# nz0001na/MorphGANformer

Hardware: AMD Instinct MI355X
Metric: latent-projection iters/sec @1024^2, k=17 latents (higher is better)
Workload: dtype f32; 1 GPU; configs[1]: single 1024x1024 face per GPU, Wing+LPIPS(squeeze)+MSE literal-mode projection step, noise_mode=random, seeded synthetic weights/targets/landmarks; k=17, z_dim=32, targets_per_gpu=1, parallelism=pair-sharded x1, graph_replay=True, loss_generator_overlap=True, steps_per_forward=32

## Files before the change

include/mgf.h:

```cpp
#ifndef MGF_H_
#define MGF_H_

#include <stdint.h>

#ifdef __cplusplus
extern "C" {
#endif

typedef void* mgf_stream_t;

enum { MGF_OK = 0, MGF_EINVAL = -1, MGF_EUNSUPPORTED = -2, MGF_ELAUNCH = -3, MGF_ETOOBIG = -4 };
enum { MGF_F32 = 0, MGF_F64 = 1, MGF_F16 = 2 };
enum { MGF_FILTER_SEPARABLE = 2 };
enum { MGF_FILTER_LARGE = 4 };
enum { MGF_ACT_LINEAR = 1, MGF_ACT_RELU = 2, MGF_ACT_LRELU = 3, MGF_ACT_TANH = 4, MGF_ACT_SIGMOID = 5,
       MGF_ACT_ELU = 6, MGF_ACT_SELU = 7, MGF_ACT_SOFTPLUS = 8, MGF_ACT_SWISH = 9,
       MGF_ACT_RELU_POST = 10 };

const char* mgf_last_error(void);
int mgf_version(void);
int mgf_device_ok(void);

int mgf_bias_act(void* y, const void* x, const void* b, const void* xref, const void* yref, const void* dy,
                 int dtype, int64_t numel, int64_t step_b, int64_t size_b,
// ... 270 lines not shown
} mgf_attn_bwd_job;
int mgf_style_demod_bwd_multi(float* dwg, const mgf_style_bwd_job* jobs_dev, int32_t njobs, int32_t n, int32_t wdim, int32_t max_channels,
                              mgf_stream_t stream);
int mgf_attn_values_bwd_multi(float* dyc, const mgf_attn_bwd_job* jobs_dev, int32_t njobs, int32_t n, int32_t t, int32_t wdim,
                              mgf_stream_t stream);
int mgf_latent_bwd_multi(float* dwg, const mgf_style_bwd_job* style_jobs_dev, int32_t n_style_jobs, float* dyc,
                         const mgf_attn_bwd_job* attn_jobs_dev, int32_t n_attn_jobs, int32_t n, int32_t t, int32_t wdim, int32_t max_channels,
                         mgf_stream_t stream);
int32_t mgf_attn_values_grad_slices(int32_t n, int32_t c, int32_t f, int32_t t);
int64_t mgf_attn_grad_job_bytes(void);
int mgf_attn_grad_multi(const void* jobs_dev, int32_t njobs, int32_t n, int32_t grad_blocks, int32_t dot_blocks, int32_t reduce_blocks,
                        mgf_stream_t stream);
int mgf_latent_grad_gather(float* dw, const float* dwg, int32_t n_style_jobs, const float* dyc, int32_t n_attn_jobs, int32_t n, int32_t k,
                           int32_t wdim, float scale, mgf_stream_t stream);
int64_t mgf_mapping_bwd_scratch_floats(int32_t k, int32_t dim, int32_t n_res_layers);
int mgf_mapping_backward(float* dz, const float* dw, const float* z, const float* params, float* scratch, int32_t n, int32_t k,
                         int32_t dim, int32_t n_res_layers, int32_t normalize_global, mgf_stream_t stream);
int mgf_mapping_forward_save(float* w, const float* z, const float* params, float* scratch, int32_t n, int32_t k, int32_t dim,
                             int32_t n_res_layers, int32_t normalize_global, mgf_stream_t stream);
int mgf_mapping_backward_saved(float* dz, const float* dw, const float* z, const float* params, float* scratch, int32_t n, int32_t k,
                               int32_t dim, int32_t n_res_layers, int32_t normalize_global, mgf_stream_t stream);

int mgf_lpips_layer_bwd_f32(float* df0, const float* f0, const float* f1_unit, const float* lin, int32_t n, int32_t c, int64_t hw,
                            int64_t f1_batch_stride, float scale, int32_t accumulate, mgf_stream_t stream);
int mgf_lpips_layer_bwd_relu_f32(float* dz_a, float* dz_b, const float* dy, const float* f0, const float* f1_unit, const float* lin,
                                 int32_t n, int32_t c, int32_t c_split, int64_t hw, int64_t f1_batch_stride, float scale,
                                 mgf_stream_t stream);
int mgf_lpips_layer_stats_f32(float* out, float* stats, const float* f0, const float* f1_unit, const float* lin, int32_t n, int32_t c,
                              int64_t hw, int64_t f1_batch_stride, int32_t accumulate, float* scratch, mgf_stream_t stream);
int mgf_lpips_layer_defer_f32(float* scratch, float* stats, const float* f0, const float* f1_unit, const float* lin, int32_t n, int32_t c, int64_t hw,
                              int64_t f1_batch_stride, int32_t* nparts_out, mgf_stream_t stream);
int mgf_lpips_finish_taps_f32(float* out, const float* scratch, int64_t set_stride_floats, int32_t ntaps, const int32_t* nparts, const float* scales,
                              int32_t n, int32_t accumulate, mgf_stream_t stream);
int mgf_lpips_layer_bwd_relu_stats_f32(float* dz_a, float* dz_b, const float* dy, const float* f0, const float* f1_unit, const float* lin,
                                       const float* stats, int32_t n, int32_t c, int32_t c_split, int64_t hw, int64_t f1_batch_stride,
                                       float scale, mgf_stream_t stream);
int mgf_relu_bwd_split_f32(float* dz_a, float* dz_b, const float* dy, const float* y, int32_t n, int32_t c, int32_t c_split, int64_t hw,
                           mgf_stream_t stream);
int mgf_maxpool3x3s2_ceil_idx_f32(float* y, uint8_t* idx, const float* x, int32_t nc, int32_t in_h, int32_t in_w, int32_t out_h,
                                  int32_t out_w, mgf_stream_t stream);
int mgf_maxpool3x3s2_ceil_bwd_idx_f32(float* dx, const float* dy, const uint8_t* idx, int32_t nc, int32_t in_h, int32_t in_w, int32_t out_h,
                                      int32_t out_w, mgf_stream_t stream);
int mgf_maxpool3x3s2_ceil_bwd_f32(float* dx, const float* dy, const float* x, int32_t nc, int32_t in_h, int32_t in_w, int32_t out_h,
                                  int32_t out_w, mgf_stream_t stream);
int mgf_maxpool_s2_floor_bwd_f32(float* dx, const float* dy, const float* x, int32_t nc, int32_t in_h, int32_t in_w, int32_t ksize,
                                 mgf_stream_t stream);
int mgf_mse_grad_f32(float* d, const float* a, const float* b, int32_t n, int64_t numel, int64_t b_batch_stride, float scale,
                     int32_t accumulate, mgf_stream_t stream);

int mgf_lpips_layer_defer_weighted_f32(float* scratch, float* stats, const float* f0, const float* f1_unit, const float* lin, const float* wmap,
                                       int32_t n, int32_t c, int64_t hw, int64_t f1_batch_stride, int64_t w_batch_stride, int32_t* nparts_out,
                                       mgf_stream_t stream);
int mgf_lpips_layer_bwd_weighted_f32(float* df0, const float* f0, const float* f1_unit, const float* lin, const float* wmap, int32_t n, int32_t c,
                                     int64_t hw, int64_t f1_batch_stride, int64_t w_batch_stride, float scale, int32_t accumulate,
                                     mgf_stream_t stream);
int mgf_lpips_layer_bwd_relu_stats_weighted_f32(float* dz_a, float* dz_b, const float* dy, const float* f0, const float* f1_unit, const float* lin,
                                                const float* stats, const float* wmap, int32_t n, int32_t c, int32_t c_split, int64_t hw,
                                                int64_t f1_batch_stride, int64_t w_batch_stride, float scale, mgf_stream_t stream);
int mgf_mse_weighted_f32(float* out, const float* a, const float* b, const float* wmap, int32_t n, int32_t c, int64_t hw, int64_t b_batch_stride,
                         int64_t w_batch_stride, float scale, int32_t accumulate, float* scratch, mgf_stream_t stream);
int mgf_mse_weighted_grad_f32(float* d, const float* a, const float* b, const float* wmap, int32_t n, int32_t c, int64_t hw,
                              int64_t b_batch_stride, int64_t w_batch_stride, float scale, int32_t accumulate, mgf_stream_t stream);

int mgf_prelu_bwd_f32(float* dx, const float* dy, const float* y, const float* slope, int32_t n, int32_t c, int64_t hw, mgf_stream_t stream);
int mgf_linear_bwd_f32(float* dx, const float* dy, const float* w, int32_t n, int32_t in_features, int32_t out_features, mgf_stream_t stream);
int mgf_resize_bilinear_bwd_f32(float* dx, const float* dy, int32_t nc, int32_t in_h, int32_t in_w, int32_t out_h, int32_t out_w,
// ... 57 lines not shown
```

morphganformer_amd/_lib.py:

```python
from __future__ import annotations

import ctypes as C
import os

import torch

HERE = os.path.dirname(os.path.abspath(__file__))
LIB_PATH = os.environ.get("MGF_LIB_PATH") or os.path.join(HERE, "libmgf_hip.so")

MGF_F32, MGF_F64, MGF_F16 = 0, 1, 2
ACT_IDS = {"linear": 1, "relu": 2, "lrelu": 3, "tanh": 4, "sigmoid": 5, "elu": 6, "selu": 7, "softplus": 8, "swish": 9,
           "relu_post": 10}
MAX_TAPS = 9

i32, i64, f32, f64, vp = C.c_int32, C.c_int64, C.c_float, C.c_double, C.c_void_p


class Epilogue(C.Structure):
    _fields_ = [("bias", vp), ("noise", vp), ("noise_strength", vp), ("noise_n", i32), ("act", i32), ("alpha", f32),
                ("gain", f32), ("residual", vp)]


class ConvDesc(C.Structure):
    _fields_ = [("n", i32), ("cin", i32), ("in_h", i32), ("in_w", i32), ("cout", i32), ("cout_pad", i32),
# ... 108 lines not shown
    "mgf_maxpool_s2_floor_f32": (C.c_int, [vp, vp, i32, i32, i32, i32, vp]),
    "mgf_maxpool3x3s2_ceil_f32": (C.c_int, [vp, vp, i32, i32, i32, i32, i32, vp]),
    "mgf_latent_perturb": (C.c_int, [vp, vp, vp, vp, vp, i32, i32, i64, vp]),
    "mgf_latent_perturb_mean": (C.c_int, [vp, vp, vp, vp, vp, i32, i32, i64, i32, vp]),
    "mgf_select_best": (C.c_int, [vp, vp, vp, vp, vp, i64, vp, vp, vp, f64, f32, vp, vp, i32, i32, vp, vp, i32, vp, vp, vp]),
    "mgf_keep_improvements": (C.c_int, [vp, vp, i64, vp, i32, vp]),
    "mgf_to_uint8_hwc": (C.c_int, [vp, vp, i32, i32, i32, vp]),
    "mgf_reference_gray_scratch_floats": (i64, []),
    "mgf_reference_gray_u8": (C.c_int, [vp, vp, i32, i32, i32, vp, vp]),
    "mgf_bwd_chunks": (i32, [i64]),
    "mgf_layer_act_bwd_f32": (C.c_int, [vp, vp, vp, vp, vp, vp, vp, vp, i32, i32, i32, i64, f32, f32, vp]),
    "mgf_channel_dot_f32": (C.c_int, [vp, vp, vp, i32, i32, i64, vp]),
    "mgf_style_grad_f32": (C.c_int, [vp, vp, vp, vp, vp, i32, i32, i64, i32, vp]),
    "mgf_style_grad_act_bwd_f32": (C.c_int, [vp, vp, vp, vp, vp, vp, vp, vp, vp, i32, vp, vp, vp, i32, i32, i32, i64, f32, f32, vp]),
    "mgf_style_act_fir_tiles": (i32, [i32, i32]),
    "mgf_style_act_fir_bwd_f32": (C.c_int, [vp, vp, vp, vp, vp, vp, vp, vp, vp, i32, vp, i32, f32, i32, i32, i32, i32, f32, f32, vp]),
    "mgf_layer_act_bwd_low_f32": (C.c_int, [vp, vp, vp, vp, vp, vp, i32, vp, vp, vp, i32, i32, i32, i64, f32, f32, vp]),
    "mgf_duplex_attention_bwd": (C.c_int, [vp, vp, vp, vp, vp, vp, vp, vp, i32, i32, i32, i32, vp]),
    "mgf_attn_values_grad": (C.c_int, [vp, vp, vp, i32, i32, i32, i32, vp]),
    "mgf_attn_values_grad_workspace_floats": (C.c_int64, [i32, i32]),
    "mgf_attn_values_grad_ws": (C.c_int, [vp, vp, vp, i32, i32, i32, i32, vp, i64, vp]),
    "mgf_style_demod_bwd_multi": (C.c_int, [vp, vp, i32, i32, i32, i32, vp]),
    "mgf_attn_values_bwd_multi": (C.c_int, [vp, vp, i32, i32, i32, i32, vp]),
    "mgf_attn_values_grad_slices": (i32, [i32, i32, i32, i32]),
    "mgf_attn_grad_job_bytes": (i64, []),
    "mgf_attn_grad_multi": (C.c_int, [vp, i32, i32, i32, i32, i32, vp]),
    "mgf_latent_bwd_multi": (C.c_int, [vp, vp, i32, vp, vp, i32, i32, i32, i32, i32, vp]),
    "mgf_latent_grad_gather": (C.c_int, [vp, vp, i32, vp, i32, i32, i32, i32, f32, vp]),
    "mgf_lpips_layer_bwd_f32": (C.c_int, [vp, vp, vp, vp, i32, i32, i64, i64, f32, i32, vp]),
    "mgf_lpips_layer_bwd_relu_f32": (C.c_int, [vp, vp, vp, vp, vp, vp, i32, i32, i32, i64, i64, f32, vp]),
    "mgf_lpips_layer_stats_f32": (C.c_int, [vp, vp, vp, vp, vp, i32, i32, i64, i64, i32, vp, vp]),
    "mgf_lpips_layer_defer_f32": (C.c_int, [vp, vp, vp, vp, vp, i32, i32, i64, i64, C.POINTER(i32), vp]),
    "mgf_lpips_finish_taps_f32": (C.c_int, [vp, vp, i64, i32, C.POINTER(i32), C.POINTER(f32), i32, i32, vp]),
    "mgf_lpips_layer_bwd_relu_stats_f32": (C.c_int, [vp, vp, vp, vp, vp, vp, vp, i32, i32, i32, i64, i64, f32, vp]),
    "mgf_relu_bwd_split_f32": (C.c_int, [vp, vp, vp, vp, i32, i32, i32, i64, vp]),
    "mgf_maxpool3x3s2_ceil_idx_f32": (C.c_int, [vp, vp, vp, i32, i32, i32, i32, i32, vp]),
    "mgf_maxpool3x3s2_ceil_bwd_idx_f32": (C.c_int, [vp, vp, vp, i32, i32, i32, i32, i32, vp]),
    "mgf_maxpool3x3s2_ceil_bwd_f32": (C.c_int, [vp, vp, vp, i32, i32, i32, i32, i32, vp]),
    "mgf_maxpool_s2_floor_bwd_f32": (C.c_int, [vp, vp, vp, i32, i32, i32, i32, vp]),
    "mgf_mse_grad_f32": (C.c_int, [vp, vp, vp, i32, i64, i64, f32, i32, vp]),
    "mgf_lpips_layer_defer_weighted_f32": (C.c_int, [vp, vp, vp, vp, vp, vp, i32, i32, i64, i64, i64, C.POINTER(i32), vp]),
    "mgf_lpips_layer_bwd_weighted_f32": (C.c_int, [vp, vp, vp, vp, vp, i32, i32, i64, i64, i64, f32, i32, vp]),
    "mgf_lpips_layer_bwd_relu_stats_weighted_f32": (C.c_int, [vp, vp, vp, vp, vp, vp, vp, vp, i32, i32, i32, i64, i64, i64, f32, vp]),
    "mgf_mse_weighted_f32": (C.c_int, [vp, vp, vp, vp, i32, i32, i64, i64, i64, f32, i32, vp, vp]),
    "mgf_mse_weighted_grad_f32": (C.c_int, [vp, vp, vp, vp, i32, i32, i64, i64, i64, f32, i32, vp]),
    "mgf_prelu_bwd_f32": (C.c_int, [vp, vp, vp, vp, i32, i32, i64, vp]),
    "mgf_linear_bwd_f32": (C.c_int, [vp, vp, vp, i32, i32, i32, vp]),
    "mgf_resize_bilinear_bwd_f32": (C.c_int, [vp, vp, i32, i32, i32, i32, i32, vp]),
    "mgf_face_crop_check": (C.c_int, [vp, i32, i32]),
    "mgf_face_crop_f32": (C.c_int, [vp, vp, vp, i32, i32, i32, i32, i32, i32, vp]),
    "mgf_face_crop_bwd_f32": (C.c_int, [vp, vp, vp, i32, i32, i32, i32, i32, i32, i32, vp]),
    "mgf_dwconv_f32": (C.c_int, [vp, vp, vp, vp, vp, vp, i32, i32, i32, i32, i32, i32, i32, i32, vp]),
    "mgf_dwconv_bwd_data_f32": (C.c_int, [vp, vp, vp, vp, vp, vp, vp, vp, i32, i32, i32, i32, i32, i32, i32, i32, vp]),
    "mgf_cv_warp_triangle_bytes": (i64, []),
    "mgf_cv_warp_triangles_f32": (C.c_int, [vp, vp, vp, vp, i32, i32, i32, i32, f32, vp]),
    "mgf_adam_step_f32": (C.c_int, [vp, vp, vp, vp, vp, vp, vp, vp, i64, i32, f32, f32, f32, f32, vp]),
    "mgf_adam_elementwise_f32": (C.c_int, [vp, vp, vp, vp, vp, vp, vp, vp, i64, i32, f32, f32, f32, f32, vp]),
    "mgf_noise_grad_f32": (C.c_int, [vp, vp, vp, i32, i64, i32, vp]),
    "mgf_noise_regularize_scratch_bytes": (i64, [i32]),
    "mgf_noise_regularize_f32": (C.c_int, [vp, vp, i32, f32, i32, vp, vp]),
    "mgf_noise_regularize_grad_f32": (C.c_int, [vp, vp, vp, i32, f32, i32, i32, vp, vp]),
    "mgf_noise_normalize_scratch_bytes": (i64, []),
    "mgf_noise_normalize_f32": (C.c_int, [vp, i64, vp, vp, i32, vp, vp]),
    "mgf_mapping_bwd_scratch_floats": (i64, [i32, i32, i32]),
    "mgf_mapping_backward": (C.c_int, [vp, vp, vp, vp, vp, i32, i32, i32, i32, i32, vp]),
    "mgf_mapping_forward_save": (C.c_int, [vp, vp, vp, vp, i32, i32, i32, i32, i32, vp]),
# ... 68 lines not shown
```

morphganformer_amd/csrc/losses.hip:

```cpp
#include "mgf_common.h"

namespace {

constexpr int RED_BLOCKS = 16384;

__device__ __forceinline__ float block_sum_256(float v, float* sm) {
    v = wave_sum(v);
    if ((threadIdx.x & 63) == 0) sm[threadIdx.x >> 6] = v;
    __syncthreads();
    float r = sm[0] + sm[1] + sm[2] + sm[3];
    __syncthreads();
    return r;
}

__global__ __launch_bounds__(256) void finish_kernel(float* out, const float* scratch, int nparts, float scale, int accumulate) {
    __shared__ float sm[4];
    const float* sc = scratch + (int64_t)blockIdx.x * RED_BLOCKS;
    float v = 0.f;
    for (int i = threadIdx.x; i < nparts; i += 256) v += sc[i];
    v = block_sum_256(v, sm);
    if (threadIdx.x == 0) out[blockIdx.x] = (accumulate ? out[blockIdx.x] : 0.f) + v * scale;
}

struct FinishSets { int nparts[8]; float scale[8]; };
__global__ __launch_bounds__(256) void finish_multi_kernel(float* out, const float* scratch, int64_t set_stride, int nsets, FinishSets fs, int accumulate) {
    __shared__ float sm[4];
    float acc = accumulate ? out[blockIdx.x] : 0.f;
    for (int t = 0; t < nsets; ++t) {
        const float* sc = scratch + (int64_t)t * set_stride + (int64_t)blockIdx.x * RED_BLOCKS;
        float v = 0.f;
        for (int i = threadIdx.x; i < fs.nparts[t]; i += 256) v += sc[i];
        v = block_sum_256(v, sm);
        acc = acc + v * fs.scale[t];
// ... 150 lines not shown
        redb[grp][px] = nb;
        redc[grp][px] = nc;
        __syncthreads();
        if (grp == 0 && valid) {
            float sb = 0.f, sc = 0.f;
#pragma unroll
            for (int g = 0; g < G; ++g) { sb += redb[g][px]; sc += redc[g][px]; }
            float* so = stats + (int64_t)nn * 3 * hw + i;
            so[0] = na; so[hw] = sb; so[2 * hw] = sc;
        }
    }
    if (MAP) {
        redb[grp][px] = d;
        __syncthreads();
        if (grp == 0 && valid) {
            float sd = 0.f;
#pragma unroll
            for (int g = 0; g < G; ++g) sd += redb[g][px];
            stats[(int64_t)nn * hw + i] = sd;
        }
        return;
    }
    if (WEIGHTED) {
        unsigned t = threadIdx.x;
        asm volatile("" : "+v"(t));
        const int64_t iw = (int64_t)blk * PXB + (int)(t % PXB);
        const __amdgpu_buffer_rsrc_t rw = __builtin_amdgcn_make_buffer_rsrc((void*)(wmap + (int64_t)nn * w_stride), 0, (int)plane_bytes, 0x00020000);
        d *= __builtin_bit_cast(float, __builtin_amdgcn_raw_buffer_load_b32(rw, 4u * (unsigned)(iw < hw ? iw : hw - 1), 0, 0));
    }
    const float acc = block_sum_256(valid ? d : 0.f, sm);
    if (threadIdx.x == 0) scratch[(int64_t)nn * RED_BLOCKS + blk] = acc;
}

template <bool UNIT_OUT>
int launch_lpips_layer(float* scratch, float* unit_out, const float* f0, const float* f1u, const float* lin, int n, int c, int64_t hw,
                       int64_t f1_stride, hipStream_t st, int* grid_out, float* stats = nullptr, float* map = nullptr,
                       const float* wmap = nullptr, int64_t w_stride = 0) {
    static const int pxb_env = [] { const char* e = mgf_knob("MGF_LPIPS_PXB"); return e ? atoi(e) : 0; }();
    const int pxb = pxb_env ? pxb_env
                  : (c <= 256 && (hw >= 65536 || (int64_t)n * mgf_cdiv(hw, 64) >= 1024)) ? 64
                  : (c > 384 && (int64_t)n * mgf_cdiv(hw, 32) >= 1024) ? 32 : 16;
    const int64_t grid64 = mgf_cdiv(hw, pxb);
    MGF_REQUIRE(grid64 <= RED_BLOCKS, MGF_ETOOBIG, "lpips_layer: %lld pixels per sample need %lld scratch floats (have %d per sample)",
                (long long)hw, (long long)grid64, RED_BLOCKS);
    MGF_REQUIRE(c <= 512, MGF_EUNSUPPORTED, "lpips_layer: at most 512 channels per tap (got %d)", c);
    MGF_REQUIRE((int64_t)c * hw < (1LL << 30), MGF_ETOOBIG, "lpips_layer: one sample's tap must stay below 4 GiB");
    MGF_REQUIRE(grid64 * n <= INT32_MAX - 8, MGF_ETOOBIG, "lpips_layer: too many workgroups");
    const int xcd_per = (int)mgf_cdiv(grid64 * n, 8);
    const dim3 grid((unsigned)(xcd_per * 8));
    *grid_out = (int)grid64;
#define MGF_LPIPS_LAUNCH(PXB, CPT)                                                                                                            \
    do {                                                                                                                                      \
        if (!UNIT_OUT && wmap && stats)                                                                                                       \
            hipLaunchKernelGGL((lpips_layer_kernel<PXB, CPT, false, true, false, true>), grid, dim3(256), 0, st, scratch, unit_out, f0, f1u,  \
                               lin, c, hw, f1_stride, n, (int)grid64, xcd_per, stats, wmap, w_stride);                                        \
        else if (!UNIT_OUT && wmap)                                                                                                           \
            hipLaunchKernelGGL((lpips_layer_kernel<PXB, CPT, false, false, false, true>), grid, dim3(256), 0, st, scratch, unit_out, f0, f1u, \
                               lin, c, hw, f1_stride, n, (int)grid64, xcd_per, nullptr, wmap, w_stride);                                      \
        else if (!UNIT_OUT && map)                                                                                                            \
            hipLaunchKernelGGL((lpips_layer_kernel<PXB, CPT, false, false, true>), grid, dim3(256), 0, st, scratch, unit_out, f0, f1u, lin, c,\
                               hw, f1_stride, n, (int)grid64, xcd_per, map, nullptr, 0);                                                      \
        else if (!UNIT_OUT && stats)                                                                                                          \
            hipLaunchKernelGGL((lpips_layer_kernel<PXB, CPT, false, true>), grid, dim3(256), 0, st, scratch, unit_out, f0, f1u, lin, c, hw,   \
                               f1_stride, n, (int)grid64, xcd_per, stats, nullptr, 0);                                                        \
        else                                                                                                                                  \
            hipLaunchKernelGGL((lpips_layer_kernel<PXB, CPT, UNIT_OUT>), grid, dim3(256), 0, st, scratch, unit_out, f0, f1u, lin, c, hw,      \
                               f1_stride, n, (int)grid64, xcd_per, nullptr, nullptr, 0);                                                      \
    } while (0)
    if (pxb == 64) {
        if (c <= 128) MGF_LPIPS_LAUNCH(64, 32); else if (c <= 256) MGF_LPIPS_LAUNCH(64, 64); else MGF_LPIPS_LAUNCH(64, 128);
    } else if (pxb == 32) {
        if (c <= 128) MGF_LPIPS_LAUNCH(32, 16); else if (c <= 256) MGF_LPIPS_LAUNCH(32, 32); else MGF_LPIPS_LAUNCH(32, 64);
    } else {
        if (c <= 128) MGF_LPIPS_LAUNCH(16, 8); else if (c <= 256) MGF_LPIPS_LAUNCH(16, 16); else MGF_LPIPS_LAUNCH(16, 32);
    }
#undef MGF_LPIPS_LAUNCH
    return MGF_OK;
}

__global__ __launch_bounds__(256) void wing_kernel(double* out, const double* pred, const double* target, int64_t numel, double omega,
                                                   double epsilon, const int32_t* pred_step, int max_row) {
    __shared__ double sm[4];
    int row = (pred_step ? *pred_step : 0) + (int)blockIdx.x;
    if (max_row >= 0 && row > max_row) row = max_row;
    pred += (int64_t)row * numel;
    const double cc = omega - omega * log(1.0 + omega / epsilon);
    double acc = 0.0;
    for (int64_t i = threadIdx.x; i < numel; i += 256) {
        double dlt = fabs(target[i] - pred[i]);
        acc += dlt < omega ? omega * log(1.0 + dlt / epsilon) : dlt - cc;
    }
    acc = wave_sum(acc);
    if ((threadIdx.x & 63) == 0) sm[threadIdx.x >> 6] = acc;
    __syncthreads();
    if (threadIdx.x == 0) out[blockIdx.x] = (sm[0] + sm[1] + sm[2] + sm[3]) / (double)numel;
}

__global__ __launch_bounds__(256) void awing_kernel(double* out, const double* pred, const double* target, int64_t numel, double omega,
                                                    double theta, double epsilon, double alpha, const int32_t* pred_step, int max_row) {
    __shared__ double sm[4];
    int row = (pred_step ? *pred_step : 0) + (int)blockIdx.x;
    if (max_row >= 0 && row > max_row) row = max_row;
    pred += (int64_t)row * numel;
    double acc = 0.0;
    for (int64_t i = threadIdx.x; i < numel; i += 256) {
        const double y = target[i];
        const double dlt = fabs(y - pred[i]);
        const double pw = alpha - y;
        if (dlt < theta) {
            acc += omega * log(1.0 + pow(dlt / omega, pw));
        } else {
            const double tp = pow(theta / epsilon, pw);
// ... 300 lines not shown
    if (rc != MGF_OK) return rc;
    MGF_CHECK_LAUNCH("lpips_unit");
    return MGF_OK;
}

extern "C" int mgf_lpips_layer_f32(float* out, const float* f0, const float* f1_unit, const float* lin, int32_t n, int32_t c, int64_t hw,
                                   int64_t f1_batch_stride, int32_t accumulate, float* scratch, mgf_stream_t stream) {
    return mgf_lpips_layer_stats_f32(out, nullptr, f0, f1_unit, lin, n, c, hw, f1_batch_stride, accumulate, scratch, stream);
}

extern "C" int mgf_lpips_layer_stats_f32(float* out, float* stats, const float* f0, const float* f1_unit, const float* lin, int32_t n, int32_t c,
                                         int64_t hw, int64_t f1_batch_stride, int32_t accumulate, float* scratch, mgf_stream_t stream) {
    MGF_REQUIRE(out && f0 && f1_unit && lin && scratch && n >= 1 && n <= 65535 && c >= 1 && hw >= 1, MGF_EINVAL, "lpips_layer: bad arguments");
    hipStream_t st = (hipStream_t)stream;
    int grid = 0;
    const int rc = launch_lpips_layer<false>(scratch, nullptr, f0, f1_unit, lin, n, c, hw, f1_batch_stride, st, &grid, stats);
    if (rc != MGF_OK) return rc;
    hipLaunchKernelGGL(finish_kernel, dim3(n), dim3(256), 0, st, out, scratch, grid, 1.0f / (float)hw, accumulate);
    MGF_CHECK_LAUNCH("lpips_layer");
    return MGF_OK;
}

extern "C" int mgf_lpips_layer_defer_f32(float* scratch, float* stats, const float* f0, const float* f1_unit, const float* lin, int32_t n, int32_t c,
                                         int64_t hw, int64_t f1_batch_stride, int32_t* nparts_out, mgf_stream_t stream) {
    MGF_REQUIRE(scratch && f0 && f1_unit && lin && nparts_out && n >= 1 && n <= 65535 && c >= 1 && hw >= 1, MGF_EINVAL, "lpips_layer_defer: bad arguments");
    int grid = 0;
    const int rc = launch_lpips_layer<false>(scratch, nullptr, f0, f1_unit, lin, n, c, hw, f1_batch_stride, (hipStream_t)stream, &grid, stats);
    if (rc != MGF_OK) return rc;
    *nparts_out = grid;
    MGF_CHECK_LAUNCH("lpips_layer_defer");
    return MGF_OK;
}

extern "C" int mgf_lpips_layer_defer_weighted_f32(float* scratch, float* stats, const float* f0, const float* f1_unit, const float* lin,
                                                  const float* wmap, int32_t n, int32_t c, int64_t hw, int64_t f1_batch_stride,
                                                  int64_t w_batch_stride, int32_t* nparts_out, mgf_stream_t stream) {
    MGF_REQUIRE(scratch && f0 && f1_unit && lin && wmap && nparts_out && n >= 1 && n <= 65535 && c >= 1 && hw >= 1 && w_batch_stride >= 0, MGF_EINVAL,
                "lpips_layer_defer_weighted: bad arguments");
    int grid = 0;
    const int rc = launch_lpips_layer<false>(scratch, nullptr, f0, f1_unit, lin, n, c, hw, f1_batch_stride, (hipStream_t)stream, &grid, stats, nullptr,
                                             wmap, w_batch_stride);
    if (rc != MGF_OK) return rc;
    *nparts_out = grid;
    MGF_CHECK_LAUNCH("lpips_layer_defer_weighted");
    return MGF_OK;
}

extern "C" int mgf_lpips_finish_taps_f32(float* out, const float* scratch, int64_t set_stride_floats, int32_t ntaps, const int32_t* nparts,
                                         const float* scales, int32_t n, int32_t accumulate, mgf_stream_t stream) {
    MGF_REQUIRE(out && scratch && nparts && scales && ntaps >= 1 && ntaps <= 8 && n >= 1 && n <= 65535, MGF_EINVAL, "lpips_finish_taps: bad arguments (1..8 taps)");
    FinishSets fs;
    for (int t = 0; t < 8; ++t) { fs.nparts[t] = t < ntaps ? nparts[t] : 0; fs.scale[t] = t < ntaps ? scales[t] : 0.f; }
    for (int t = 0; t < ntaps; ++t) MGF_REQUIRE(nparts[t] >= 1 && nparts[t] <= RED_BLOCKS, MGF_EINVAL, "lpips_finish_taps: bad partial count");
    hipLaunchKernelGGL(finish_multi_kernel, dim3(n), dim3(256), 0, (hipStream_t)stream, out, scratch, set_stride_floats, ntaps, fs, accumulate);
    MGF_CHECK_LAUNCH("lpips_finish_taps");
    return MGF_OK;
}

extern "C" int mgf_lpips_layer_map_f32(float* map, const float* f0, const float* f1_unit, const float* lin, int32_t n, int32_t c, int64_t hw,
                                       int64_t f1_batch_stride, mgf_stream_t stream) {
    MGF_REQUIRE(map && f0 && f1_unit && lin && n >= 1 && n <= 65535 && c >= 1 && hw >= 1, MGF_EINVAL, "lpips_layer_map: bad arguments");
    int grid = 0;
    const int rc = launch_lpips_layer<false>(nullptr, nullptr, f0, f1_unit, lin, n, c, hw, f1_batch_stride, (hipStream_t)stream, &grid, nullptr, map);
    if (rc != MGF_OK) return rc;
    MGF_CHECK_LAUNCH("lpips_layer_map");
    return MGF_OK;
// ... 581 lines not shown
```

morphganformer_amd/lpips.py:

```python
from __future__ import annotations

import ctypes as C
import math
import os

import numpy as np
import torch

from . import _lib
from . import lpips_backbones as backbones
from .lpips_backbones import (ALEX_SPEC, CHNS, FIRES, NET_CHNS, POOLS, SCALE, SHIFT, SPECS, TAPS_AFTER, VGG_SPEC,
                              SequentialFeatures, SqueezeFeatures, _pool_out, load_backbone_state, random_backbone, random_squeeze_backbone)

WEIGHTS_DIR = os.path.join(os.path.dirname(os.path.abspath(__file__)), "weights")


def region_tap_weights(weight, sides):
    w = torch.as_tensor(weight).to(torch.float64)
    lead = w.shape[:-2]
    w4 = w.reshape(-1, 1, *w.shape[-2:])
    out = []
    for hh, ww in sides:
        wl = torch.nn.functional.adaptive_avg_pool2d(w4, (int(hh), int(ww)))
        wl = wl / wl.sum(dim=(2, 3), keepdim=True)
# ... 139 lines not shown
        if tuple(target_a.shape) != tuple(target_b.shape):
            raise ValueError(f"set_target_pair: the two targets differ in shape: {tuple(target_a.shape)} vs {tuple(target_b.shape)}")
        n = int(target_a.shape[0])
        al = np.asarray(alpha.detach().cpu() if isinstance(alpha, torch.Tensor) else alpha, dtype=np.float64).reshape(-1)
        if al.size not in (1, n) or not np.all((al >= 0.0) & (al <= 1.0)):
            raise ValueError(f"set_target_pair: alpha must be one value or {n} values in [0, 1] (got {alpha!r})")
        al = np.array(np.broadcast_to(al, (n,)))
        buf = self._pair_offset_buf
        if buf is None or buf.numel() != n:
            buf = self._pair_offset_buf = torch.zeros(n, dtype=torch.float32, device=self.device_)
        self.set_target(target_b)
        ub = [t.clone() for t in self._target_taps]
        self.distance_into(buf, target_a.float().contiguous())
        buf.mul_(torch.as_tensor(al * (1.0 - al), dtype=torch.float32, device=self.device_))
        self.set_target(target_a)
        for t, b in zip(self._target_taps, ub):
            for i in range(n):
                a = float(al[i])
                if a == 1.0:
                    t[i].copy_(b[i])
                elif a != 0.0:
                    t[i].mul_(1.0 - a).add_(b[i], alpha=a)
        self.pair_offset = buf

    def grad_into(self, dimg, scale=1.0, accumulate=False):
        f = self._last
        assert f is not None and tuple(dimg.shape) == (f.n, 3, *self._last_hw), "call distance_into(..., keep_taps=True) first"
        g = f.backward(self._target_taps, self.lins, scale, per_sample=self._target_n > 1, region=self._region_for(f.n, *self._last_hw))
        if not accumulate:
            dimg.zero_()
        dimg[:, :, :g.shape[2], :g.shape[3]].add_(g)
        return dimg

    def _forward_taps(self, pred, keep_taps=False, out=None, scalar=True):
        n, _, h, w = pred.shape
        f = self._features(n, h, w)
        assert self._target_taps is not None, "call set_target first"
        per_sample = self._target_n > 1
        assert not per_sample or self._target_n == n, f"{self._target_n} targets cannot pair with {n} candidates"
        if scalar:
            need = n * int(_lib.lib().mgf_reduce_scratch_floats())
            if self._scratch.numel() < need:
                self._scratch = torch.empty(need, dtype=torch.float32, device=self.device_)
            if out is None:
                out = torch.zeros(len(self.chns), n, dtype=torch.float32, device=self.device_)
        if keep_taps is not None:
            self._last, self._last_hw = (f, (h, w)) if keep_taps else (None, None)
        f.tap_stats = {}
        region = self._region_for(n, h, w) if scalar else None
        if scalar and self.fused_stem and not keep_taps and not per_sample and region is None:
            f.stem(pred.contiguous(), feat_ref=self._target_taps[0], lin=self.lins[0], dist_out=out if out.dim() == 1 else out[0],
                   scratch=self._scratch)
            taps = f(pred, from_pooled=True)
        else:
            taps = f(pred, argmax=True) if (keep_taps and self.net == "squeeze") else f(pred)
        return f, taps, per_sample, region, out

    def _defer_tap(self, i, a, scratch, stats, per_sample, region):
        n, c, hh, ww = a.shape
        L, st, hw, got = _lib.lib(), _lib.stream_ptr(), hh * ww, C.c_int32(0)
        maps = (a.data_ptr(), self._target_taps[i].data_ptr(), self.lins[i].data_ptr())
        if region is not None:
            _lib.check(L.mgf_lpips_layer_defer_weighted_f32(scratch.data_ptr(), _lib.ptr(stats), *maps, region[0][i].data_ptr(), n, c, hw,
                                                            c * hw if per_sample else 0, hw if region[1] > 1 else 0, C.byref(got), st),
                       "lpips_layer_weighted")
            return got.value, 1.0
        _lib.check(L.mgf_lpips_layer_defer_f32(scratch.data_ptr(), _lib.ptr(stats), *maps, n, c, hw, c * hw if per_sample else 0, C.byref(got), st),
                   "lpips_layer")
        return got.value, 1.0 / float(hw)

    def distance_into(self, out, pred, keep_taps=False):
        f, taps, per_sample, region, _ = self._forward_taps(pred, bool(keep_taps), out)
        n = pred.shape[0]
        L, st = _lib.lib(), _lib.stream_ptr()
        red = int(L.mgf_reduce_scratch_floats())
        ntaps = len(self.lins)
        if self._scratch.numel() < ntaps * n * red:
            self._scratch = torch.empty(ntaps * n * red, dtype=torch.float32, device=self.device_)
        nparts, scales, k, first_done = (C.c_int32 * 8)(), (C.c_float * 8)(), 0, False
        for i, a in enumerate(taps):
            if a is None:
                first_done = True
                continue
            hw = a.shape[2] * a.shape[3]
            stats = None
            if keep_taps and backbones.TAP_STATS:
                key = (i, n, hw)
                stats = self._stats.get(key)
                if stats is None:
                    stats = self._stats[key] = torch.empty(n, 3, hw, dtype=torch.float32, device=self.device_)
                f.tap_stats[i] = stats
            nparts[k], scales[k] = self._defer_tap(i, a, self._scratch[k * n * red:], stats, per_sample, region)
            k += 1
        _lib.check(L.mgf_lpips_finish_taps_f32(out.data_ptr(), self._scratch.data_ptr(), n * red, k, nparts, scales, n, int(first_done), st),
                   "lpips_finish_taps")
        return out

    def distance_per_tap(self, pred):
        f, taps, per_sample, region, out = self._forward_taps(pred, None)
        n = pred.shape[0]
        L, st = _lib.lib(), _lib.stream_ptr()
        for i, (a, b, lin) in enumerate(zip(taps, self._target_taps, self.lins)):
            if a is None:
                continue
            _, c, hh, ww = a.shape
            if region is not None:
                nparts, scale = self._defer_tap(i, a, self._scratch, None, per_sample, region)
                _lib.check(L.mgf_lpips_finish_taps_f32(out[i].data_ptr(), self._scratch.data_ptr(), n * int(L.mgf_reduce_scratch_floats()), 1,
                                                       (C.c_int32 * 8)(nparts), (C.c_float * 8)(scale), n, 0, st), "lpips_finish_taps")
                continue
            _lib.check(L.mgf_lpips_layer_stats_f32(out[i].data_ptr(), None, a.data_ptr(), b.data_ptr(), lin.data_ptr(), n, c, hh * ww,
                                                   c * hh * ww if per_sample else 0, 0, self._scratch.data_ptr(), st), "lpips_layer")
        return out

    @staticmethod
    def _require_square(H, W):
        if H != W:
            raise _lib.MgfError(f"PerceptualLoss(spatial=True): the image must be square (got {H}x{W}): the reference derives ONE scale factor from "
                                "the height and its tap maps then disagree in width")

    def _map_workspace(self, n, H, f):
        ws = self._map_ws.get((n, H))
        if ws is None:
            sides = []
            for l, (_, hh, ww) in enumerate(f.tap_shapes):
                got = spatial_tap_output_side(hh, H)
                if hh != ww or got != H:
# ... 66 lines not shown
```

morphganformer_amd/lpips_backbones.py:

```python
from __future__ import annotations

import math
import os

import numpy as np
import torch

from . import _lib
from . import conv as cv

FIRES = {3: (64, 16, 64), 4: (128, 16, 64), 6: (128, 32, 128), 7: (256, 32, 128),
         9: (256, 48, 192), 10: (384, 48, 192), 11: (384, 64, 256), 12: (512, 64, 256)}
TAPS_AFTER = [1, 4, 7, 9, 10, 11, 12]
POOLS = [2, 5, 8]
CHNS = [64, 128, 256, 384, 384, 512, 512]
SHIFT = (-0.030, -0.088, -0.188)
SCALE = (0.458, 0.448, 0.450)
USE_WINOGRAD_LPIPS = os.environ.get("MGF_WINOGRAD_LPIPS", "1") != "0"
FUSE_TAP_RELU = os.environ.get("MGF_FUSE_TAP_RELU", "1") != "0"
POOL_ARGMAX = os.environ.get("MGF_POOL_ARGMAX", "1") != "0"
TAP_STATS = os.environ.get("MGF_TAP_STATS", "1") != "0"
MERGE_FIRE = os.environ.get("MGF_LPIPS_MERGE_FIRE", "1") != "0"


def random_squeeze_backbone(seed=0):
    rng = np.random.Generator(np.random.PCG64(seed))
    sd = {}

    def conv(name, co, ci, k):
        sd[name + ".weight"] = (rng.standard_normal((co, ci, k, k)) * math.sqrt(2.0 / (ci * k * k))).astype(np.float32)
        sd[name + ".bias"] = (rng.standard_normal(co) * 0.05).astype(np.float32)

    conv("features.0", 64, 3, 3)
    for idx, (ci, sq, ex) in FIRES.items():
        conv(f"features.{idx}.squeeze", sq, ci, 1)
        conv(f"features.{idx}.expand1x1", ex, sq, 1)
        conv(f"features.{idx}.expand3x3", ex, sq, 3)
    return sd


VGG_SPEC = ([("conv", 0, 3, 64, 3, 1, 1), ("conv", 2, 64, 64, 3, 1, 1), ("tap",), ("pool", 2),
             ("conv", 5, 64, 128, 3, 1, 1), ("conv", 7, 128, 128, 3, 1, 1), ("tap",), ("pool", 2),
             ("conv", 10, 128, 256, 3, 1, 1), ("conv", 12, 256, 256, 3, 1, 1), ("conv", 14, 256, 256, 3, 1, 1), ("tap",), ("pool", 2),
             ("conv", 17, 256, 512, 3, 1, 1), ("conv", 19, 512, 512, 3, 1, 1), ("conv", 21, 512, 512, 3, 1, 1), ("tap",), ("pool", 2),
             ("conv", 24, 512, 512, 3, 1, 1), ("conv", 26, 512, 512, 3, 1, 1), ("conv", 28, 512, 512, 3, 1, 1), ("tap",)])
ALEX_SPEC = ([("conv", 0, 3, 64, 11, 4, 2), ("tap",), ("pool", 3), ("conv", 3, 64, 192, 5, 1, 2), ("tap",), ("pool", 3),
              ("conv", 6, 192, 384, 3, 1, 1), ("tap",), ("conv", 8, 384, 256, 3, 1, 1), ("tap",), ("conv", 10, 256, 256, 3, 1, 1), ("tap",)])
SPECS = {"vgg": VGG_SPEC, "alex": ALEX_SPEC}
NET_CHNS = {"squeeze": CHNS, "vgg": [64, 128, 256, 512, 512], "alex": [64, 192, 384, 256, 256]}


def random_backbone(net, seed=0):
    if net == "squeeze":
        return random_squeeze_backbone(seed)
    rng = np.random.Generator(np.random.PCG64(seed))
# ... 291 lines not shown
            sqT, e1T, e3T = self.gp[idx]
            da, db = self.gex[idx]
            if not fused:
                self._relu_bwd(gh, h, da, db)
            s, gs = self.sq[idx], self.gsq[idx]
            merged = idx in self.merge
            if merged:
                gc = self.gcat[idx]
                if idx in self.gpwm and min(hh, ww) > 16 and cv.winograd_fills_chip(n, gs.shape[1], hh, ww):
                    cv.winograd_forward(gc, self.gpwm[idx], out=gs)
                else:
                    cv.conv_forward(gc, self.gpm[idx], pad=(1, 1), out=gs)
            else:
                cv.conv_forward(da, e1T, out=gs)
            if merged:
                pass
            elif idx in self.gpw and cv.winograd_fills_chip(n, gs.shape[1], hh, ww):
                cv.winograd_forward(db, self.gpw[idx], epilogue=_lib.make_epilogue(residual=gs), out=gs)
            else:
                cv.conv_forward(db, e3T, pad=(1, 1), epilogue=_lib.make_epilogue(residual=gs), out=gs)
            self._relu_bwd(gs, s)
            cv.conv_forward(gs, sqT, out=self.gbufs[idx - 1])
        raise AssertionError("unreachable")

    def stem(self, x, feat_out=None, feat_ref=None, lin=None, dist_out=None, scratch=None):
        _lib.require_gpu(x, feat_out, feat_ref, dist_out)
        n, _, h, w = x.shape
        assert n == self.n and x.is_contiguous() and x.dtype == torch.float32
        _lib.check(_lib.lib().mgf_lpips_stem_f32(self.buf[2].data_ptr(), x.data_ptr(), self.stem_w.data_ptr(), self.stem_b.data_ptr(),
                                                 _lib.ptr(feat_out), _lib.ptr(feat_ref), _lib.ptr(lin), _lib.ptr(dist_out), n, h, w, 0,
                                                 _lib.ptr(scratch), _lib.stream_ptr()), "lpips_stem")
        return self.buf[2]

    def __call__(self, x, out=None, from_pooled=False, argmax=False):
        _lib.require_gpu(x)
        L = _lib.lib()
        st = _lib.stream_ptr()
        taps = []
        self.have_argmax = bool(argmax) and not from_pooled and POOL_ARGMAX

        def dest(idx):
            if idx in TAPS_AFTER and out is not None:
                return out[TAPS_AFTER.index(idx)]
            return self.buf[idx]

        if from_pooled:
            h = self.buf[2]
            taps.append(None)
        else:
            pc, b = self.c0
            if cv.NARROW_CONV:
                h = cv.conv3x3s2_few_inputs(x.contiguous(), self.stem_w.view(64, 3, 3, 3), bias=b, relu=True, out=dest(1))
            else:
                h = cv.conv_forward(x.contiguous(), pc, stride=2, pad=(0, 0), epilogue=_lib.make_epilogue(bias=b, act="relu"), out=dest(1))
            taps.append(h)
        for idx in range(3 if from_pooled else 2, 13):
            if idx in POOLS:
                y = self.buf[idx]
                n, c, ih, iw = h.shape
                if self.have_argmax:
                    if idx not in self.pidx:
                        self.pidx[idx] = torch.empty(y.shape, dtype=torch.uint8, device=y.device)
                    _lib.check(L.mgf_maxpool3x3s2_ceil_idx_f32(y.data_ptr(), self.pidx[idx].data_ptr(), h.data_ptr(), n * c, ih, iw, y.shape[2],
                                                               y.shape[3], st), "maxpool_idx")
                else:
                    _lib.check(L.mgf_maxpool3x3s2_ceil_f32(y.data_ptr(), h.data_ptr(), n * c, ih, iw, y.shape[2], y.shape[3], st), "maxpool")
                h = y
            else:
                (ps, bs), (p1, b1), (p3, b3) = self.fires[idx]
                s = cv.conv_forward(h, ps, epilogue=_lib.make_epilogue(bias=bs, act="relu"), out=self.sq[idx])
                y = dest(idx)
                ex = p1.cout
                if idx in self.merge:
                    cv.winograd2_forward(s, self.wino3m[idx], epilogue=_lib.make_epilogue(bias=self.merged[idx][1], act="relu"), out=y)
                    h = y
                    if idx in TAPS_AFTER:
                        taps.append(h)
                    continue
                cv.conv_forward(s, p1, epilogue=_lib.make_epilogue(bias=b1, act="relu"), out=y, out_choff=0)
                if idx in self.wino3 and min(s.shape[2:]) > 16 and cv.winograd_fills_chip(s.shape[0], ex, s.shape[2], s.shape[3]):
                    cv.winograd2_forward(s, self.wino3[idx], epilogue=_lib.make_epilogue(bias=b3, act="relu"), out=y, out_choff=ex)
                else:
                    cv.conv_forward(s, p3, pad=(1, 1), epilogue=_lib.make_epilogue(bias=b3, act="relu"), out=y, out_choff=ex)
                h = y
            if idx in TAPS_AFTER:
                taps.append(h)
        return taps
```

Baseline: 798.9 iters/s.

## Fuse LPIPS tap distance reduction with following 3x3 stride-2 maxpool

Adds a HIP kernel that reads a SqueezeNet tap feature map once and, in the same pass, computes the normalized LPIPS distance partial sums and writes the 3x3/s2 ceil max-pooled output using DPP row maxes and buffer loads. The Python forward path calls it in place of the separate maxpool and deferred tap-distance kernels whenever a pool directly follows a tap, argmax is off and there is no region. The aim is to avoid reading the large tap activations twice. Scratch indexing changes to per-tap slots, so the finish call is offset by the fused-stem slot. The cost is a complex tiled kernel with halo rows and columns and hand-written inline asm.

Result: no change. 798.4 iters/s (median of 4 runs) (-0.1%).

```diff
diff --git a/include/mgf.h b/include/mgf.h
--- a/include/mgf.h
+++ b/include/mgf.h
@@ -326,6 +326,9 @@
                               int64_t f1_batch_stride, int32_t* nparts_out, mgf_stream_t stream);
 int mgf_lpips_finish_taps_f32(float* out, const float* scratch, int64_t set_stride_floats, int32_t ntaps, const int32_t* nparts, const float* scales,
                               int32_t n, int32_t accumulate, mgf_stream_t stream);
+int mgf_lpips_layer_pool_defer_f32(float* scratch, float* pooled, const float* f0, const float* f1_unit, const float* lin, int32_t n, int32_t c,
+                                   int32_t h, int32_t w, int32_t oh, int32_t ow, int64_t f1_batch_stride, int32_t* nparts_out,
+                                   mgf_stream_t stream);
 int mgf_lpips_layer_bwd_relu_stats_f32(float* dz_a, float* dz_b, const float* dy, const float* f0, const float* f1_unit, const float* lin,
                                        const float* stats, int32_t n, int32_t c, int32_t c_split, int64_t hw, int64_t f1_batch_stride,
                                        float scale, mgf_stream_t stream);
diff --git a/morphganformer_amd/_lib.py b/morphganformer_amd/_lib.py
--- a/morphganformer_amd/_lib.py
+++ b/morphganformer_amd/_lib.py
@@ -164,6 +164,7 @@
     "mgf_lpips_layer_stats_f32": (C.c_int, [vp, vp, vp, vp, vp, i32, i32, i64, i64, i32, vp, vp]),
     "mgf_lpips_layer_defer_f32": (C.c_int, [vp, vp, vp, vp, vp, i32, i32, i64, i64, C.POINTER(i32), vp]),
     "mgf_lpips_finish_taps_f32": (C.c_int, [vp, vp, i64, i32, C.POINTER(i32), C.POINTER(f32), i32, i32, vp]),
+    "mgf_lpips_layer_pool_defer_f32": (C.c_int, [vp, vp, vp, vp, vp, i32, i32, i32, i32, i32, i32, i64, C.POINTER(i32), vp]),
     "mgf_lpips_layer_bwd_relu_stats_f32": (C.c_int, [vp, vp, vp, vp, vp, vp, vp, i32, i32, i32, i64, i64, f32, vp]),
     "mgf_relu_bwd_split_f32": (C.c_int, [vp, vp, vp, vp, i32, i32, i32, i64, vp]),
     "mgf_maxpool3x3s2_ceil_idx_f32": (C.c_int, [vp, vp, vp, i32, i32, i32, i32, i32, vp]),
diff --git a/morphganformer_amd/csrc/losses.hip b/morphganformer_amd/csrc/losses.hip
--- a/morphganformer_amd/csrc/losses.hip
+++ b/morphganformer_amd/csrc/losses.hip
@@ -1,4 +1,6 @@
 #include "mgf_common.h"
+#include <algorithm>
+#include <type_traits>
 
 namespace {
 
@@ -215,14 +217,18 @@
     if (threadIdx.x == 0) scratch[(int64_t)nn * RED_BLOCKS + blk] = acc;
 }
 
+int lpips_pxb(int n, int c, int64_t hw) {
+    static const int pxb_env = [] { const char* e = mgf_knob("MGF_LPIPS_PXB"); return e ? atoi(e) : 0; }();
+    return pxb_env ? pxb_env
+         : (c <= 256 && (hw >= 65536 || (int64_t)n * mgf_cdiv(hw, 64) >= 1024)) ? 64
+         : (c > 384 && (int64_t)n * mgf_cdiv(hw, 32) >= 1024) ? 32 : 16;
+}
+
 template <bool UNIT_OUT>
 int launch_lpips_layer(float* scratch, float* unit_out, const float* f0, const float* f1u, const float* lin, int n, int c, int64_t hw,
                        int64_t f1_stride, hipStream_t st, int* grid_out, float* stats = nullptr, float* map = nullptr,
                        const float* wmap = nullptr, int64_t w_stride = 0) {
-    static const int pxb_env = [] { const char* e = mgf_knob("MGF_LPIPS_PXB"); return e ? atoi(e) : 0; }();
-    const int pxb = pxb_env ? pxb_env
-                  : (c <= 256 && (hw >= 65536 || (int64_t)n * mgf_cdiv(hw, 64) >= 1024)) ? 64
-                  : (c > 384 && (int64_t)n * mgf_cdiv(hw, 32) >= 1024) ? 32 : 16;
+    const int pxb = lpips_pxb(n, c, hw);
     const int64_t grid64 = mgf_cdiv(hw, pxb);
     MGF_REQUIRE(grid64 <= RED_BLOCKS, MGF_ETOOBIG, "lpips_layer: %lld pixels per sample need %lld scratch floats (have %d per sample)",
                 (long long)hw, (long long)grid64, RED_BLOCKS);
@@ -261,6 +267,145 @@
     return MGF_OK;
 }
 
+struct TapPoolParams {
+    float* scratch; float* pooled; const float* f0; const float* f1u; const float* lin;
+    int64_t f1_stride;
+    int n, c, h, w, oh, ow, tiles_x, stride, bands, K, xcd_per;
+};
+
+__device__ __forceinline__ float tp_vmax(float a, float b) { float d; asm("v_max_f32 %0, %1, %2" : "=v"(d) : "v"(a), "v"(b)); return d; }
+#define TP_DPP " wave_shl:1 row_mask:0xf bank_mask:0xf\n\t"
+__device__ __forceinline__ void tp_hmax3_x4(float& x0, float& x1, float& x2, float& x3) {
+    float m0, m1, m2, m3;
+    asm volatile("s_nop 1\n\t"
+                 "v_max_f32_dpp %4, %0, %0" TP_DPP "v_max_f32_dpp %5, %1, %1" TP_DPP
+                 "v_max_f32_dpp %6, %2, %2" TP_DPP "v_max_f32_dpp %7, %3, %3" TP_DPP
+                 "v_max_f32_dpp %0, %4, %4" TP_DPP "v_max_f32_dpp %1, %5, %5" TP_DPP
+                 "v_max_f32_dpp %2, %6, %6" TP_DPP "v_max_f32_dpp %3, %7, %7" TP_DPP
+                 : "+v"(x0), "+v"(x1), "+v"(x2), "+v"(x3), "=&v"(m0), "=&v"(m1), "=&v"(m2), "=&v"(m3));
+}
+#undef TP_DPP
+
+template <int W, int CPT, int NCLS>
+__global__ __launch_bounds__(64 * W) void lpips_tap_pool_kernel(TapPoolParams p) {
+    constexpr int G = W * NCLS;
+    static_assert(CPT % 4 == 0 && CPT % NCLS == 0, "channels per wave: whole DPP quads, whole rounds of lane groups");
+    __shared__ float red[2][G][64];
+    __shared__ float lin_s[W * CPT];
+    __shared__ float sm[W];
+    const int lane = threadIdx.x & 63;
+    const int g = __builtin_amdgcn_readfirstlane((int)(threadIdx.x >> 6));
+    int item = (blockIdx.x & 7) * p.xcd_per + (blockIdx.x >> 3);
+    if (item >= p.n * p.tiles_x * p.bands) return;
+    const int tx = item % p.tiles_x; item /= p.tiles_x;
+    const int nn = item % p.n, band = item / p.n;
+    for (int i = threadIdx.x; i < W * CPT; i += 64 * W) lin_s[i] = i < p.c ? p.lin[i] : 0.f;
+
+    const int hw = p.h * p.w, ohw = p.oh * p.ow;
+    const unsigned plane_bytes = 4u * (unsigned)hw, oplane_bytes = 4u * (unsigned)ohw;
+    const __amdgpu_buffer_rsrc_t ra = __builtin_amdgcn_make_buffer_rsrc((void*)(p.f0 + (int64_t)nn * p.c * hw), 0, (int)((unsigned)p.c * plane_bytes), 0x00020000);
+    const __amdgpu_buffer_rsrc_t rb = __builtin_amdgcn_make_buffer_rsrc((void*)(p.f1u + (int64_t)nn * p.f1_stride), 0, (int)((unsigned)p.c * plane_bytes), 0x00020000);
+    const __amdgpu_buffer_rsrc_t rp = __builtin_amdgcn_make_buffer_rsrc((void*)(p.pooled + (int64_t)nn * p.c * ohw), 0, (int)((unsigned)p.c * oplane_bytes), 0x00020000);
+    const int x0 = tx * p.stride;
+    const bool last_tx = tx == p.tiles_x - 1, last_band = band == p.bands - 1;
+    const int ncols = last_tx ? p.w - x0 : p.stride + 2;
+    const bool colvalid = lane < ncols;
+    const bool colown = last_tx ? colvalid : lane < p.stride;
+    const int ox = (x0 >> 1) + (lane >> 1);
+    const bool emit_lane = !(lane & 1) && colown && ox < p.ow;
+    const unsigned rec_in = (unsigned)p.c * plane_bytes, rec_out = (unsigned)p.c * oplane_bytes;
+    const unsigned vo = colvalid ? (unsigned)g * plane_bytes + 4u * (unsigned)(x0 + lane) : rec_in;
+    const unsigned vp = emit_lane ? (unsigned)g * oplane_bytes + 4u * (unsigned)ox : rec_out;
+    const int oy0 = band * p.K, r0 = 2 * oy0;
+    const float NEG = -3.0e38f;
+
+    float P[CPT];
+    float dsum = 0.f;
+    int buf = 0;
+    __syncthreads();
+
+    auto load_row = [&](const __amdgpu_buffer_rsrc_t rsrc, const int rr, const bool wanted, float (&x)[CPT]) {
+        const int ro = (int)(4u * (unsigned)((r0 + rr) * p.w));
+        unsigned vx = wanted ? vo : rec_in;
+        asm volatile("" : "+v"(vx));
+#pragma unroll
+        for (int j = 0; j < CPT; ++j)
+            x[j] = __builtin_bit_cast(float, __builtin_amdgcn_raw_buffer_load_b32(rsrc, vx + (unsigned)(j * W) * plane_bytes, ro, 0));
+    };
+    auto row_ok = [&](const int rr) { return rr <= 2 * p.K && r0 + rr < p.h; };
+    auto row_own = [&](const int rr) { return row_ok(rr) && (rr < 2 * p.K || last_band); };
+    auto step = [&](const int rr, auto odd_tag) {
+        constexpr bool ODD = decltype(odd_tag)::value;
+        const bool ok = row_ok(rr), own = row_own(rr);
+        float u[CPT], v[CPT];
+        load_row(ra, rr, ok, u);
+        load_row(rb, rr, own, v);
+        float na[NCLS];
+#pragma unroll
+        for (int a = 0; a < NCLS; ++a) na[a] = 0.f;
+#pragma unroll
+        for (int j = 0; j < CPT; ++j) na[j % NCLS] += u[j] * u[j];
+#pragma unroll
+        for (int a = 0; a < NCLS; ++a) red[buf][g + W * a][lane] = na[a];
+        __syncthreads();
+        if (own) {
+            float nt = 0.f;
+#pragma unroll
+            for (int gg = 0; gg < G; ++gg) nt += red[buf][gg][lane];
+            const float ia = 1.f / (sqrtf(nt) + 1e-10f);
+            float d = 0.f;
+#pragma unroll
+            for (int j = 0; j < CPT; ++j) {
+                const float ua = u[j] * ia;
+                const float e = ua - v[j];
+                d += lin_s[g + j * W] * e * e;
+            }
+            dsum += d;
+        }
+        buf ^= 1;
+        if (!ok || last_tx) {
+            const bool pm = ok && colvalid;
+#pragma unroll
+            for (int j = 0; j < CPT; ++j) u[j] = pm ? u[j] : NEG;
+        }
+#pragma unroll
+        for (int j = 0; j < CPT; j += 4) tp_hmax3_x4(u[j], u[j + 1], u[j + 2], u[j + 3]);
+        if (ODD) {
+#pragma unroll
+            for (int j = 0; j < CPT; ++j) P[j] = tp_vmax(P[j], u[j]);
+        } else {
+            if (rr > 0) {
+                const int oy = oy0 + (rr >> 1) - 1;
+                unsigned vs = oy < p.oh ? vp : rec_out;
+                asm volatile("" : "+v"(vs));
+                const int oo = (int)(4u * (unsigned)(oy * p.ow));
+#pragma unroll
+                for (int j = 0; j < CPT; ++j)
+                    __builtin_amdgcn_raw_buffer_store_b32(__builtin_bit_cast(unsigned, tp_vmax(P[j], u[j])), rp, vs + (unsigned)(j * W) * oplane_bytes, oo, 0);
+            }
+#pragma unroll
+            for (int j = 0; j < CPT; ++j) P[j] = u[j];
+        }
+    };
+    step(0, std::false_type{});
+    for (int i = 0; i < p.K; ++i) {
+        if (r0 + 2 * i + 1 >= p.h) break;
+        step(2 * i + 1, std::true_type{});
+        step(2 * i + 2, std::false_type{});
+    }
+    dsum = wave_sum(colown ? dsum : 0.f);
+    if (lane == 0) sm[g] = dsum;
+    __syncthreads();
+    if (threadIdx.x == 0) {
+        float acc = 0.f;
+#pragma unroll
+        for (int gg = 0; gg < W; ++gg) acc += sm[gg];
+        p.scratch[(int64_t)nn * RED_BLOCKS + band * p.tiles_x + tx] = acc;
+    }
+}
+
+int tap_pool_out(int in) { int o = (in - 3 + 1) / 2 + 1; if ((o - 1) * 2 >= in) --o; return o; }
+
 __global__ __launch_bounds__(256) void wing_kernel(double* out, const double* pred, const double* target, int64_t numel, double omega,
                                                    double epsilon, const int32_t* pred_step, int max_row) {
     __shared__ double sm[4];
@@ -627,6 +772,51 @@
     return MGF_OK;
 }
 
+extern "C" int mgf_lpips_layer_pool_defer_f32(float* scratch, float* pooled, const float* f0, const float* f1_unit, const float* lin, int32_t n,
+                                              int32_t c, int32_t h, int32_t w, int32_t oh, int32_t ow, int64_t f1_batch_stride, int32_t* nparts_out,
+                                              mgf_stream_t stream) {
+    MGF_REQUIRE(scratch && pooled && f0 && f1_unit && lin && nparts_out && n >= 1 && n <= 65535 && c >= 1 && f1_batch_stride >= 0, MGF_EINVAL,
+                "lpips_layer_pool_defer: bad arguments");
+    MGF_REQUIRE(h >= 3 && w >= 3, MGF_EINVAL, "lpips_layer_pool_defer: the map must be at least 3x3 (got %dx%d)", h, w);
+    MGF_REQUIRE(oh == tap_pool_out(h) && ow == tap_pool_out(w), MGF_EINVAL, "lpips_layer_pool_defer: pooled map must be %dx%d (got %dx%d)",
+                tap_pool_out(h), tap_pool_out(w), oh, ow);
+    MGF_REQUIRE(c <= 512, MGF_EUNSUPPORTED, "lpips_layer_pool_defer: at most 512 channels per tap (got %d)", c);
+    const int64_t hw = (int64_t)h * w;
+    MGF_REQUIRE((int64_t)(c + (c <= 128 ? 128 : c <= 256 ? 256 : 512)) * hw < (1LL << 30), MGF_ETOOBIG,
+                "lpips_layer_pool_defer: one sample's tap, padded to 128 / 256 / 512 channels more, must stay below 4 GiB");
+    TapPoolParams p;
+    p.scratch = scratch; p.pooled = pooled; p.f0 = f0; p.f1u = f1_unit; p.lin = lin; p.f1_stride = f1_batch_stride;
+    p.n = n; p.c = c; p.h = h; p.w = w; p.oh = oh; p.ow = ow;
+    p.tiles_x = (int)std::max<int64_t>(1, mgf_cdiv(w - 2, 60));
+    p.stride = 2 * (int)mgf_cdiv(mgf_cdiv(w - 2, p.tiles_x), 2);
+    if (p.tiles_x > 1 && w - p.stride * (p.tiles_x - 1) < 3) p.stride = 60;
+    p.K = (int)std::min<int64_t>(8, std::max<int64_t>(2, mgf_cdiv(oh, 16)));
+    p.bands = (int)mgf_cdiv(oh, p.K);
+    const int64_t per_sample = (int64_t)p.tiles_x * p.bands;
+    MGF_REQUIRE(per_sample <= RED_BLOCKS, MGF_ETOOBIG, "lpips_layer_pool_defer: a %dx%d map needs %lld scratch floats per sample (have %d)", h, w,
+                (long long)per_sample, RED_BLOCKS);
+    MGF_REQUIRE(per_sample * n <= INT32_MAX - 8, MGF_ETOOBIG, "lpips_layer_pool_defer: too many workgroups");
+    p.xcd_per = (int)mgf_cdiv(per_sample * n, 8);
+    const dim3 grid((unsigned)(p.xcd_per * 8));
+    const int G = 256 / lpips_pxb(1, c, hw);
+    const int cpad = c <= 128 ? 128 : c <= 256 ? 256 : 512;
+    const int W = std::min(G, cpad / 32), cpt = cpad / W, ncls = G / W;
+#define MGF_TAP_POOL(WW, CC, NC) hipLaunchKernelGGL((lpips_tap_pool_kernel<WW, CC, NC>), grid, dim3(64 * WW), 0, (hipStream_t)stream, p)
+    if (W == 4 && cpt == 32 && ncls == 4) MGF_TAP_POOL(4, 32, 4);
+    else if (W == 8 && cpt == 32 && ncls == 2) MGF_TAP_POOL(8, 32, 2);
+    else if (W == 16 && cpt == 32 && ncls == 1) MGF_TAP_POOL(16, 32, 1);
+    else if (W == 4 && cpt == 32 && ncls == 2) MGF_TAP_POOL(4, 32, 2);
+    else if (W == 8 && cpt == 32 && ncls == 1) MGF_TAP_POOL(8, 32, 1);
+    else if (W == 8 && cpt == 64 && ncls == 1) MGF_TAP_POOL(8, 64, 1);
+    else if (W == 4 && cpt == 32 && ncls == 1) MGF_TAP_POOL(4, 32, 1);
+    else if (W == 4 && cpt == 64 && ncls == 1) MGF_TAP_POOL(4, 64, 1);
+    else MGF_REQUIRE(false, MGF_EUNSUPPORTED, "lpips_layer_pool_defer: no kernel for %d lane groups and %d channels", G, c);
+#undef MGF_TAP_POOL
+    *nparts_out = (int)per_sample;
+    MGF_CHECK_LAUNCH("lpips_layer_pool_defer");
+    return MGF_OK;
+}
+
 extern "C" int mgf_lpips_layer_defer_weighted_f32(float* scratch, float* stats, const float* f0, const float* f1_unit, const float* lin,
                                                   const float* wmap, int32_t n, int32_t c, int64_t hw, int64_t f1_batch_stride,
                                                   int64_t w_batch_stride, int32_t* nparts_out, mgf_stream_t stream) {
diff --git a/morphganformer_amd/lpips.py b/morphganformer_amd/lpips.py
--- a/morphganformer_amd/lpips.py
+++ b/morphganformer_amd/lpips.py
@@ -195,7 +195,7 @@
         dimg[:, :, :g.shape[2], :g.shape[3]].add_(g)
         return dimg
 
-    def _forward_taps(self, pred, keep_taps=False, out=None, scalar=True):
+    def _forward_taps(self, pred, keep_taps=False, out=None, scalar=True, tap_pool=None):
         n, _, h, w = pred.shape
         f = self._features(n, h, w)
         assert self._target_taps is not None, "call set_target first"
@@ -211,12 +211,15 @@
             self._last, self._last_hw = (f, (h, w)) if keep_taps else (None, None)
         f.tap_stats = {}
         region = self._region_for(n, h, w) if scalar else None
+        if tap_pool is not None and (self.net != "squeeze" or keep_taps or region is not None):
+            tap_pool = None
+        fuse = {} if tap_pool is None else {"tap_pool": lambda i, a, y: tap_pool(i, a, y, per_sample)}
         if scalar and self.fused_stem and not keep_taps and not per_sample and region is None:
             f.stem(pred.contiguous(), feat_ref=self._target_taps[0], lin=self.lins[0], dist_out=out if out.dim() == 1 else out[0],
                    scratch=self._scratch)
-            taps = f(pred, from_pooled=True)
-        else:
-            taps = f(pred, argmax=True) if (keep_taps and self.net == "squeeze") else f(pred)
+            taps = f(pred, from_pooled=True, **fuse)
+        else:
+            taps = f(pred, argmax=True) if (keep_taps and self.net == "squeeze") else f(pred, **fuse)
         return f, taps, per_sample, region, out
 
     def _defer_tap(self, i, a, scratch, stats, per_sample, region):
@@ -233,17 +236,31 @@
         return got.value, 1.0 / float(hw)
 
     def distance_into(self, out, pred, keep_taps=False):
-        f, taps, per_sample, region, _ = self._forward_taps(pred, bool(keep_taps), out)
         n = pred.shape[0]
         L, st = _lib.lib(), _lib.stream_ptr()
         red = int(L.mgf_reduce_scratch_floats())
         ntaps = len(self.lins)
         if self._scratch.numel() < ntaps * n * red:
             self._scratch = torch.empty(ntaps * n * red, dtype=torch.float32, device=self.device_)
-        nparts, scales, k, first_done = (C.c_int32 * 8)(), (C.c_float * 8)(), 0, False
+        pooled_taps = {}
+
+        def tap_pool(i, a, y, per_sample):
+            _, c, hh, ww = a.shape
+            got = C.c_int32(0)
+            _lib.check(L.mgf_lpips_layer_pool_defer_f32(self._scratch[i * n * red:].data_ptr(), y.data_ptr(), a.data_ptr(),
+                                                        self._target_taps[i].data_ptr(), self.lins[i].data_ptr(), n, c, hh, ww, y.shape[2], y.shape[3],
+                                                        c * hh * ww if per_sample else 0, C.byref(got), st), "lpips_layer_pool")
+            pooled_taps[i] = (got.value, 1.0 / float(hh * ww))
+
+        f, taps, per_sample, region, _ = self._forward_taps(pred, bool(keep_taps), out, tap_pool=tap_pool)
+        nparts, scales, k, first = (C.c_int32 * 8)(), (C.c_float * 8)(), 0, 0
         for i, a in enumerate(taps):
             if a is None:
-                first_done = True
+                first = 1
+                continue
+            if i in pooled_taps:
+                nparts[k], scales[k] = pooled_taps[i]
+                k += 1
                 continue
             hw = a.shape[2] * a.shape[3]
             stats = None
@@ -253,9 +270,9 @@
                 if stats is None:
                     stats = self._stats[key] = torch.empty(n, 3, hw, dtype=torch.float32, device=self.device_)
                 f.tap_stats[i] = stats
-            nparts[k], scales[k] = self._defer_tap(i, a, self._scratch[k * n * red:], stats, per_sample, region)
+            nparts[k], scales[k] = self._defer_tap(i, a, self._scratch[i * n * red:], stats, per_sample, region)
             k += 1
-        _lib.check(L.mgf_lpips_finish_taps_f32(out.data_ptr(), self._scratch.data_ptr(), n * red, k, nparts, scales, n, int(first_done), st),
+        _lib.check(L.mgf_lpips_finish_taps_f32(out.data_ptr(), self._scratch[first * n * red:].data_ptr(), n * red, k, nparts, scales, n, first, st),
                    "lpips_finish_taps")
         return out
 
diff --git a/morphganformer_amd/lpips_backbones.py b/morphganformer_amd/lpips_backbones.py
--- a/morphganformer_amd/lpips_backbones.py
+++ b/morphganformer_amd/lpips_backbones.py
@@ -21,6 +21,7 @@
 POOL_ARGMAX = os.environ.get("MGF_POOL_ARGMAX", "1") != "0"
 TAP_STATS = os.environ.get("MGF_TAP_STATS", "1") != "0"
 MERGE_FIRE = os.environ.get("MGF_LPIPS_MERGE_FIRE", "1") != "0"
+TAP_POOL = os.environ.get("MGF_LPIPS_TAP_POOL", "1") != "0"
 
 
 def random_squeeze_backbone(seed=0):
@@ -378,7 +379,7 @@
                                                  _lib.ptr(scratch), _lib.stream_ptr()), "lpips_stem")
         return self.buf[2]
 
-    def __call__(self, x, out=None, from_pooled=False, argmax=False):
+    def __call__(self, x, out=None, from_pooled=False, argmax=False, tap_pool=None):
         _lib.require_gpu(x)
         L = _lib.lib()
         st = _lib.stream_ptr()
@@ -404,7 +405,9 @@
             if idx in POOLS:
                 y = self.buf[idx]
                 n, c, ih, iw = h.shape
-                if self.have_argmax:
+                if tap_pool is not None and TAP_POOL and not self.have_argmax and idx > 2 and idx - 1 in TAPS_AFTER:
+                    tap_pool(len(taps) - 1, h, y)
+                elif self.have_argmax:
                     if idx not in self.pidx:
                         self.pidx[idx] = torch.empty(y.shape, dtype=torch.uint8, device=y.device)
                     _lib.check(L.mgf_maxpool3x3s2_ceil_idx_f32(y.data_ptr(), self.pidx[idx].data_ptr(), h.data_ptr(), n * c, ih, iw, y.shape[2],
```
